# wen-yuan-zhang/Fast-Learning-NeRF

Measured on AMD Instinct MI355X. Metric: training rays/sec (Lego-like 800x800, 64+128 samples) + PSNR@N-iters, higher is better.
Workload: dtype f32; 1 GPU; nerf-ours Lego full 800x800 (BASELINE configs[1]), SURVEY 8(d) throughput protocol: 4096 uniformly drawn rays per GPU per step, 64+128 samples, use_viewdirs, white_bkgd, perturb=1, U[0,1) targets, random-init nets, leaf-error table on, fp32-width bf16x6 kernels, plain backward (FASTNERF_COMPACT=0); parallelism=dp1, math_mode=bf16x6, backward=plain (every sample)

## Files before the change

fast-learning-nerf_amd/csrc/mlp_bwd_dw.hip:

```cpp
#include "mlp_common.h"
#include "dw_pair.h"
#include <atomic>

int fn_launch_dx(int mm, int grid, hipStream_t st, int64_t P, const float* draw, const float* act, const float* params, const float* packed_bwd,
                 float* dact, const NetLayout& L, const int* live_idx, const int* live_cnt, float* headws, int flags);

#define DW_MT 32

template <int WO, int WI, int TO, int TI, bool BIAS, bool RANK1>
__global__ void __launch_bounds__(WO * WI * 64, WO * WI / 4)
mlp_bwd_dw_kernel(int64_t P, const float* __restrict__ dY, int ldy, const float* __restrict__ X, int ldx,
                  const float* __restrict__ draw , float* __restrict__ partial_w,
                  float* __restrict__ partial_b, float* __restrict__ partial_r, const int* __restrict__ live_idx,
                  const int* __restrict__ live_cnt) {
  if (live_idx) P = (int64_t)__builtin_amdgcn_readfirstlane(*live_cnt);
  constexpr int NO = WO * TO * 32, KI = WI * TI * 32;
  constexpr int NTD = WO * WI * 64;
  constexpr int STAGE = DW_MT * (NO + KI) + DW_MT;
  extern __shared__ __attribute__((aligned(16))) float smem[];
  const int tid = threadIdx.x;
  const int lane = tid & 63;
  const int wave = __builtin_amdgcn_readfirstlane(tid >> 6);
  const int wo = wave / WI, wi = wave % WI;
  const int64_t ntile_all = (P + DW_MT - 1) / DW_MT;
  const int64_t per = (ntile_all + gridDim.x - 1) / gridDim.x;
  const int64_t t0 = blockIdx.x * per;
  int64_t t1 = t0 + per;
  if (t1 > ntile_all) t1 = ntile_all;

  f32x16 acc[TO][TI];
#pragma unroll
  for (int a = 0; a < TO; ++a)
#pragma unroll
    for (int b = 0; b < TI; ++b)
#pragma unroll
      for (int r = 0; r < 16; ++r) acc[a][b][r] = 0.f;
  float bsum = 0.f, rsum = 0.f;

  constexpr int YV = (DW_MT * NO / 4 + NTD - 1) / NTD;
  constexpr int XV = (DW_MT * KI / 4 + NTD - 1) / NTD;
  static_assert(DW_MT * NO % 4 == 0 && DW_MT * KI % 4 == 0 && NO <= NTD && KI <= NTD, "stage split");
  float4 ry[YV], rx[XV];
  float rda = 0.f;

  auto load_stage = [&](int64_t t) {
    const int64_t pbase = t * DW_MT;
#pragma unroll
    for (int i = 0; i < YV; ++i) {
      const int e = (i * NTD + tid) * 4;
      const int m = e / NO, c = e % NO;
      const int64_t p = pbase + m;
      ry[i] = (e < DW_MT * NO && p < P) ? *reinterpret_cast<const float4*>(dY + p * ldy + c)
                                        : make_float4(0.f, 0.f, 0.f, 0.f);
    }
#pragma unroll
    for (int i = 0; i < XV; ++i) {
      const int e = (i * NTD + tid) * 4;
      const int m = e / KI, c = e % KI;
      const int64_t p = pbase + m;
      rx[i] = (e < DW_MT * KI && p < P) ? *reinterpret_cast<const float4*>(X + p * ldx + c)
                                        : make_float4(0.f, 0.f, 0.f, 0.f);
    }
    if (RANK1 && tid < DW_MT) {
      const int64_t p = pbase + tid;
      rda = (p < P) ? draw[(live_idx ? (int64_t)live_idx[p] : p) * 4 + 3] : 0.f;
    }
  };
  auto store_stage = [&](float* st) {
#pragma unroll
    for (int i = 0; i < YV; ++i)
      if ((i * NTD + tid) * 4 < DW_MT * NO) *reinterpret_cast<float4*>(st + (i * NTD + tid) * 4) = ry[i];
#pragma unroll
    for (int i = 0; i < XV; ++i)
      if ((i * NTD + tid) * 4 < DW_MT * KI) *reinterpret_cast<float4*>(st + DW_MT * NO + (i * NTD + tid) * 4) = rx[i];
    if (RANK1 && tid < DW_MT) st[DW_MT * (NO + KI) + tid] = rda;
  };

  if (t0 < t1) {
    load_stage(t0);
    store_stage(smem);
  }
  __syncthreads();
  for (int64_t t = t0; t < t1; ++t) {
    float* cur = smem + ((t - t0) & 1) * STAGE;
    float* nxt = smem + (((t - t0) & 1) ^ 1) * STAGE;
    if (t + 1 < t1) load_stage(t + 1);
    const float* Ys = cur;
    const float* Xs = cur + DW_MT * NO;
    {
      float fa0[TO], fb0[TI], fa1[TO], fb1[TI];
      auto ldf = [&](float (&a)[TO], float (&b)[TI], int k2) {
        const int m = k2 * 2 + (lane >> 5);
#pragma unroll
        for (int i = 0; i < TO; ++i) a[i] = Ys[m * NO + (wo * TO + i) * 32 + (lane & 31)];
#pragma unroll
        for (int j = 0; j < TI; ++j) b[j] = Xs[m * KI + (wi * TI + j) * 32 + (lane & 31)];
      };
      auto mm = [&](const float (&a)[TO], const float (&b)[TI]) {
#pragma unroll
        for (int i = 0; i < TO; ++i)
#pragma unroll
          for (int j = 0; j < TI; ++j) acc[i][j] = mfma(a[i], b[j], acc[i][j]);
      };
      ldf(fa0, fb0, 0);
#pragma unroll
      for (int k2 = 0; k2 < DW_MT / 2; k2 += 2) {
        ldf(fa1, fb1, k2 + 1);
        __builtin_amdgcn_sched_barrier(0);
        mm(fa0, fb0);
        __builtin_amdgcn_sched_barrier(0);
        if (k2 + 2 < DW_MT / 2) ldf(fa0, fb0, k2 + 2);
        __builtin_amdgcn_sched_barrier(0);
        mm(fa1, fb1);
        __builtin_amdgcn_sched_barrier(0);
      }
    }
    if (BIAS) {
      if (tid < NO) {
#pragma unroll 8
        for (int m = 0; m < DW_MT; ++m) bsum += Ys[m * NO + tid];
      }
    }
    if (RANK1) {
      if (tid < KI) {
        const float* da = cur + DW_MT * (NO + KI);
#pragma unroll 8
        for (int m = 0; m < DW_MT; ++m) rsum = fmaf(da[m], Xs[m * KI + tid], rsum);
      }
    }
    if (t + 1 < t1) store_stage(nxt);
    __syncthreads();
  }
  float* pw = partial_w + (int64_t)blockIdx.x * NO * KI;
#pragma unroll
  for (int i = 0; i < TO; ++i)
#pragma unroll
    for (int j = 0; j < TI; ++j)
#pragma unroll
      for (int r = 0; r < 16; ++r) {
        const int o = (wo * TO + i) * 32 + crow(r, lane);
        const int c = (wi * TI + j) * 32 + (lane & 31);
        pw[(int64_t)o * KI + c] = acc[i][j][r];
      }
  if (BIAS && tid < NO) partial_b[(int64_t)blockIdx.x * NO + tid] = bsum;
  if (RANK1 && tid < KI) partial_r[(int64_t)blockIdx.x * KI + tid] = rsum;
}

template <int WO, int WI, int TO, int TI, bool BIAS, bool RANK1, int CTI2 = 0, int CTO2 = 0, bool RBV = false>
__device__ __forceinline__ void dw6_body(const int64_t P, const float* __restrict__ dY, const float* __restrict__ X,
                                         const float* __restrict__ draw, float* __restrict__ partial_w, float* __restrict__ partial_b,
                                         float* __restrict__ partial_r, const int* __restrict__ live_idx,
                                         const float* __restrict__ X2, const float* __restrict__ dY2, const int wg, const int nwg,
                                         const float* __restrict__ rb_wr = nullptr) {
  constexpr int NO = WO * TO * 32, KI = WI * TI * 32;
  constexpr int CTO = WO * TO, CTI = WI * TI, NTILE = CTO + CTI;
  constexpr int NW = WO * WI;
  constexpr int TPW = (NTILE + NW - 1) / NW;
  extern __shared__ __attribute__((aligned(16))) uint4 S6[];
  float* const DA = reinterpret_cast<float*>(S6 + 2 * NTILE * 192);
  float4* const DR = reinterpret_cast<float4*>(DA + 32);
  static_assert(!RBV || (RANK1 && CTO2 == 0), "the view job: draw is staged, one gradient tensor");
  const int tid = threadIdx.x;
  const int lane = tid & 63;
  const int wave = __builtin_amdgcn_readfirstlane(tid >> 6);
  const int wo = wave / WI, wi = wave % WI;
  const int64_t nq_all = (P + 15) / 16;
  const int64_t per = (nq_all + nwg - 1) / nwg;
  const int64_t q0 = wg * per;
  int64_t q1 = q0 + per;
  if (q1 > nq_all) q1 = nq_all;
  const int nq = (int)(q1 - q0);
  int64_t Pend = q1 * 16;
  if (Pend > P) Pend = P;

  f32x16 acc[TO][TI];
#pragma unroll
  for (int a = 0; a < TO; ++a)
#pragma unroll
    for (int b = 0; b < TI; ++b)
#pragma unroll
      for (int r = 0; r < 16; ++r) acc[a][b][r] = 0.f;
  float ssum[TPW];
#pragma unroll
  for (int k = 0; k < TPW; ++k) ssum[k] = 0.f;

  constexpr int CTI1 = CTI - CTI2, KI1 = CTI1 * 32, KI2 = CTI2 * 32;
  constexpr int CTO1 = CTO - CTO2, NO1 = CTO1 * 32, NO2 = CTO2 * 32;
  static_assert(!(RANK1 && CTO2) && !(CTI2 && CTO2), "one second tensor per job");
  const float* tsrc[TPW];
  bool tisy[TPW], tis2[TPW];
  constexpr bool KNOWN = (CTO % NW == 0) && (NTILE % NW == 0) && CTO2 == 0 && CTI2 == 0;
#pragma unroll
  for (int k = 0; k < TPW; ++k) {
    const int t = k * NW + wave;
    tisy[k] = KNOWN ? (k * NW < CTO) : (t < CTO);
    tis2[k] = (CTI2 > 0 && t >= CTO + CTI1) || (CTO2 > 0 && t >= CTO1 && t < CTO);
    tsrc[k] = tisy[k] ? (tis2[k] ? dY2 + q0 * (16 * NO2) + (t - CTO1) * 32 : dY + q0 * (16 * NO1) + t * 32)
                      : (tis2[k] ? X2 + q0 * (16 * KI2) + (t - CTO - CTI1) * 32 : X + q0 * (16 * KI1) + (t - CTO) * 32);
  }
  const int relmax = (int)(Pend - q0 * 16) - 1;
  const int col = lane & 31, half8 = (lane >> 5) * 8;
  const unsigned boffy = (unsigned)(half8 * NO1 + col) * 4u, boffy2 = (unsigned)(half8 * NO2 + col) * 4u,
                 boffx = (unsigned)(half8 * KI1 + col) * 4u, boffx2 = (unsigned)(half8 * KI2 + col) * 4u;
  struct Raw { float v[TPW][8]; };
  float wr0[TPW], wr1[TPW], wr2[TPW];
  if constexpr (RBV) {
#pragma unroll
    for (int k = 0; k < TPW; ++k) {
      const int t = k * NW + wave;
      if (tisy[k] && (NTILE % NW == 0 || t < NTILE)) {
        wr0[k] = rb_wr[t * 32 + col]; wr1[k] = rb_wr[128 + t * 32 + col]; wr2[k] = rb_wr[256 + t * 32 + col];
      } else {
        wr0[k] = wr1[k] = wr2[k] = 0.f;
      }
    }
  }
  auto ldb = [](const float* base, unsigned byte_off) __attribute__((always_inline)) -> float {
    return *reinterpret_cast<const float*>(reinterpret_cast<const char*>(base) + byte_off);
  };
  auto load_raw = [&](Raw& r, int st, auto whole) __attribute__((always_inline)) {
    if constexpr (decltype(whole)::value) {
#pragma unroll
      for (int k = 0; k < TPW; ++k) {
        const int t = k * NW + wave;
        if (NTILE % NW == 0 || t < NTILE) {
          if (tisy[k] && CTO2 > 0 && tis2[k]) {
            const float* b = tsrc[k] + (int64_t)st * (16 * NO2);
#pragma unroll
            for (int e = 0; e < 8; ++e) r.v[k][e] = ldb(b, boffy2 + (unsigned)(e * NO2 * 4));
          } else if (tisy[k]) {
            const float* b = tsrc[k] + (int64_t)st * (16 * NO1);
#pragma unroll
            for (int e = 0; e < 8; ++e) r.v[k][e] = ldb(b, boffy + (unsigned)(e * NO1 * 4));
          } else if (CTI2 > 0 && tis2[k]) {
            const float* b = tsrc[k] + (int64_t)st * (16 * KI2);
#pragma unroll
            for (int e = 0; e < 8; ++e) r.v[k][e] = ldb(b, boffx2 + (unsigned)(e * KI2 * 4));
          } else {
            const float* b = tsrc[k] + (int64_t)st * (16 * KI1);
#pragma unroll
            for (int e = 0; e < 8; ++e) r.v[k][e] = ldb(b, boffx + (unsigned)(e * KI1 * 4));
          }
        }
      }
    } else {
      unsigned row[8];
#pragma unroll
      for (int e = 0; e < 8; ++e) { const int rr = st * 16 + half8 + e; row[e] = (unsigned)(rr < relmax ? rr : relmax); }
#pragma unroll
      for (int k = 0; k < TPW; ++k) {
        const int t = k * NW + wave;
        if (NTILE % NW == 0 || t < NTILE) {
#pragma unroll
          for (int e = 0; e < 8; ++e)
            r.v[k][e] = ldb(tsrc[k], (row[e] * (unsigned)(tisy[k] ? (tis2[k] ? NO2 : NO1) : (tis2[k] ? KI2 : KI1)) + (unsigned)col) * 4u);
        }
      }
    }
  };
  const int* const li = live_idx ? live_idx : reinterpret_cast<const int*>(draw);
  auto load_ix = [&](int st) __attribute__((always_inline)) -> int64_t {
    const int rr = st * 16 + (lane & 15);
    const int64_t p = q0 * 16 + (rr < relmax ? rr : relmax);
    const int64_t lv = li[p];
    return live_idx ? lv : p;
  };
  auto split_store = [&](const Raw& r, int buf, int st, auto whole) __attribute__((always_inline)) {
    const int nv = relmax + 1 - (st * 16 + half8);
#pragma unroll
    for (int k = 0; k < TPW; ++k) {
      const int t = k * NW + wave;
      if (NTILE % NW == 0 || t < NTILE) {
        float v[8];
#pragma unroll
        for (int e = 0; e < 8; ++e) v[e] = r.v[k][e];
        if constexpr (RBV) {
          if (tisy[k]) {
#pragma unroll
            for (int e = 0; e < 8; ++e) {
              const float4 d = DR[(st & 1) * 16 + half8 + e];
              v[e] = dyv_value(v[e], d.x, d.y, d.z, wr0[k], wr1[k], wr2[k]);
            }
          }
        }
        if constexpr (!decltype(whole)::value) {
#pragma unroll
          for (int e = 0; e < 8; ++e) v[e] = e < nv ? v[e] : 0.f;
        }
        uint4 h, m, l;
        uint4* d = S6 + ((buf * NTILE + t) * 3) * 64 + lane;
        split3_frag(make_float4(v[0], v[1], v[2], v[3]), make_float4(v[4], v[5], v[6], v[7]), h, m, l);
        d[0] = h; d[64] = m; d[128] = l;
        if (BIAS && (KNOWN ? (k * NW < CTO) : (t < CTO1))) ssum[k] += ((v[0] + v[1]) + (v[2] + v[3])) + ((v[4] + v[5]) + (v[6] + v[7]));
        if (RANK1 && (KNOWN ? (k * NW >= CTO) : (t >= CTO && t < CTO + CTI1))) {
          const float4 d0 = *reinterpret_cast<const float4*>(DA + (st & 1) * 16 + half8);
          const float4 d1 = *reinterpret_cast<const float4*>(DA + (st & 1) * 16 + half8 + 4);
          const float da[8] = {d0.x, d0.y, d0.z, d0.w, d1.x, d1.y, d1.z, d1.w};
#pragma unroll
          for (int e = 0; e < 8; ++e) ssum[k] = fmaf(da[e], v[e], ssum[k]);
        }
      }
    }
  };
  auto multiply = [&](int buf) __attribute__((always_inline)) {
    const uint4* Sb = S6 + buf * NTILE * 192 + lane;
    uint4 a[TO][3];
#pragma unroll
    for (int i = 0; i < TO; ++i)
#pragma unroll
      for (int pl = 0; pl < 3; ++pl) a[i][pl] = Sb[((wo * TO + i) * 3 + pl) * 64];
    constexpr int PA[6] = {2, 0, 1, 1, 0, 0}, PB[6] = {0, 2, 1, 0, 1, 0};
    constexpr int JP = TI >= 2 ? 2 : 1;
#pragma unroll
    for (int j0 = 0; j0 < TI; j0 += JP) {
      uint4 b[JP][3];
#pragma unroll
      for (int jj = 0; jj < JP; ++jj)
#pragma unroll
        for (int pl = 0; pl < 3; ++pl)
          if (j0 + jj < TI) b[jj][pl] = Sb[((CTO + wi * TI + j0 + jj) * 3 + pl) * 64];
#pragma unroll
      for (int t = 0; t < 6; ++t)
#pragma unroll
        for (int jj = 0; jj < JP; ++jj)
#pragma unroll
          for (int i = 0; i < TO; ++i)
            if (j0 + jj < TI) acc[i][j0 + jj] = mfma_bf16(a[i][PA[t]], b[jj][PB[t]], acc[i][j0 + jj]);
    }
  };
  auto publish = [&]() __attribute__((always_inline)) {
    asm volatile("s_waitcnt lgkmcnt(0)\n\ts_barrier" ::: "memory");
  };

  if (nq > 0) {
    constexpr std::true_type WHOLE{};
    constexpr std::false_type ANY{};
    Raw r0, r1;
    load_raw(r0, 0, ANY);
    load_raw(r1, 1, ANY);
    typedef typename std::conditional<RBV, float4, float>::type DrawT;
    auto ld_draw = [&](int64_t ix) __attribute__((always_inline)) -> DrawT {
      if constexpr (RBV) return *reinterpret_cast<const float4*>(draw + ix * 4);
      else return draw[ix * 4 + 3];
    };
    auto st_draw = [&](int slot, const DrawT& d) __attribute__((always_inline)) {
      if constexpr (RBV) { DA[slot] = d.w; DR[slot] = d; }
      else DA[slot] = d;
    };
    DrawT dr0 = DrawT(), dr1 = DrawT();
    int64_t ix0 = 0, ix1 = 0;
    const bool da_lane = RANK1 && wave == 0 && lane < 16;
    if (da_lane) {
      st_draw(lane, ld_draw(load_ix(0)));
      st_draw(16 + lane, ld_draw(load_ix(1)));
      dr0 = ld_draw(load_ix(2));
      dr1 = ld_draw(load_ix(3));
      ix0 = load_ix(4);
      ix1 = load_ix(5);
    }
    if (RANK1) publish();
    split_store(r0, 0, 0, ANY);
    load_raw(r0, 2, ANY);
    publish();
    auto mix = [&](auto sync) __attribute__((always_inline)) {
      if constexpr (KNOWN && !RANK1) interleave6<0, TO * TI * 6, TPW * 4 * 11 + (BIAS ? 8 : 0), decltype(sync)::value>();
    };
    auto pair = [&](int d, auto whole) __attribute__((always_inline)) {
      const int st = 2 * d;
      if (da_lane) { st_draw(lane, dr0); dr0 = ld_draw(ix0); ix0 = load_ix(st + 6); }
      multiply(0);
      split_store(r1, 1, st + 1, whole);
      mix(std::integral_constant<int, 1>{});
      load_raw(r1, st + 3, whole);
      publish();
      if (da_lane) { st_draw(16 + lane, dr1); dr1 = ld_draw(ix1); ix1 = load_ix(st + 7); }
      multiply(1);
      split_store(r0, 0, st + 2, whole);
      mix(std::integral_constant<int, 2>{});
      load_raw(r0, st + 4, whole);
      publish();
    };
    const int n2 = (nq + 1) / 2;
    const int nwhole = (relmax + 1) / 16;
    int dmain = nwhole >= 5 ? (nwhole - 3) / 2 : 0;
    if (dmain > n2) dmain = n2;
#pragma unroll 1
    for (int d = 0; d < dmain; ++d) pair(d, WHOLE);
#pragma unroll 1
    for (int d = dmain; d < n2; ++d) pair(d, ANY);
  }
  float* pw = partial_w + (int64_t)wg * NO * KI;
#pragma unroll
  for (int i = 0; i < TO; ++i)
#pragma unroll
    for (int j = 0; j < TI; ++j)
#pragma unroll
      for (int r = 0; r < 16; ++r) {
        const int o = (wo * TO + i) * 32 + crow(r, lane);
        const int c = (wi * TI + j) * 32 + (lane & 31);
        pw[(int64_t)o * KI + c] = acc[i][j][r];
      }
  if (BIAS || RANK1) {
#pragma unroll
    for (int k = 0; k < TPW; ++k) {
      const int t = k * NW + wave;
      if (NTILE % NW == 0 || t < NTILE) {
        const float sv = ssum[k] + __shfl_xor(ssum[k], 32, 64);
        if (lane < 32) {
          if (BIAS && t < CTO1) partial_b[(int64_t)wg * NO1 + t * 32 + lane] = sv;
          if (RANK1 && t >= CTO && t < CTO + CTI1) partial_r[(int64_t)wg * KI1 + (t - CTO) * 32 + lane] = sv;
        }
      }
    }
  }
}

template <int WO, int WI, int TO, int TI, bool BIAS, bool RANK1, int CTI2 = 0, int CTO2 = 0>
__global__ void __launch_bounds__(WO * WI * 64, WO * WI / 4)
mlp_bwd_dw6_kernel(int64_t P, const float* __restrict__ dY, const float* __restrict__ X,
                   const float* __restrict__ draw, float* __restrict__ partial_w, float* __restrict__ partial_b,
                   float* __restrict__ partial_r, const int* __restrict__ live_idx, const int* __restrict__ live_cnt,
                   const float* __restrict__ X2 = nullptr, const float* __restrict__ dY2 = nullptr) {
  if (live_idx) P = (int64_t)__builtin_amdgcn_readfirstlane(*live_cnt);
  dw6_body<WO, WI, TO, TI, BIAS, RANK1, CTI2, CTO2>(P, dY, X, draw, partial_w, partial_b, partial_r, live_idx, X2, dY2, (int)blockIdx.x,
                                                    (int)gridDim.x);
}

template <int WO, int WI, int TO, int TI, bool BIAS, bool RANK1, int CTI2>
__global__ void __launch_bounds__(WO * WI * 64, WO * WI / 4)
mlp_bwd_dw6_rbv_kernel(int64_t P, const float* __restrict__ hv, const float* __restrict__ X, const float* __restrict__ draw,
                       float* __restrict__ partial_w, float* __restrict__ partial_b, float* __restrict__ partial_r,
                       const float* __restrict__ X2, const float* __restrict__ wr) {
  dw6_body<WO, WI, TO, TI, BIAS, RANK1, CTI2, 0, true>(P, hv, X, draw, partial_w, partial_b, partial_r, nullptr, X2, nullptr, (int)blockIdx.x,
                                                       (int)gridDim.x, wr);
}

#define DW_QMAX 256
__host__ __device__ static inline int dw_trunk_chunks(int64_t P, int ncu) {
  const int unit = ncu >= 8 ? ncu / 8 : 1;
  const int64_t nq = (P + 15) / 16;
  int64_t k = (nq + (int64_t)unit * DW_QMAX - 1) / ((int64_t)unit * DW_QMAX);
  k = k < 1 ? 1 : (k > 8 ? 8 : k);
  return unit * (int)k;
}
__global__ void __launch_bounds__(512, 2)
mlp_bwd_dw6_trunk_kernel(int64_t P, DwTrunk J, const int* __restrict__ live_idx, const int* __restrict__ live_cnt, int ncu) {
  if (live_idx) P = (int64_t)__builtin_amdgcn_readfirstlane(*live_cnt);
  const int nact = dw_trunk_chunks(P, ncu);
  if ((int)blockIdx.x >= nact) return;
  const int job = (int)blockIdx.y;
  dw6_body<4, 2, 2, 4, true, false>(P, J.dY[job], J.X[job], nullptr, J.pw[job], J.pb[job], nullptr, live_idx, nullptr, nullptr,
                                    (int)blockIdx.x, nact);
}

struct DwTrunkPair {
  DwTrunk J[2];
  int64_t P[2];
};
__global__ void __launch_bounds__(512, 2)
mlp_bwd_dw6_trunk_pair_kernel(DwTrunkPair A, int ncu) {
  const int c0 = dw_trunk_chunks(A.P[0], ncu);
  int b = (int)blockIdx.x;
  const int pass = b >= DW_TRUNK_JOBS * c0 ? 1 : 0;
  if (pass) b -= DW_TRUNK_JOBS * c0;
  const int64_t P = A.P[pass];
  const int nact = pass ? dw_trunk_chunks(P, ncu) : c0;
  const int job = b / nact;
  if (job >= DW_TRUNK_JOBS) return;
  const DwTrunk& J = A.J[pass];
  dw6_body<4, 2, 2, 4, true, false>(P, J.dY[job], J.X[job], nullptr, J.pw[job], J.pb[job], nullptr, nullptr, nullptr, nullptr, b - job * nact,
                                    nact);
}

__global__ void __launch_bounds__(128) head_grads_kernel(int64_t P, const float* __restrict__ draw,
                                                          const float* __restrict__ hv,
                                                          float* __restrict__ partial, const int* __restrict__ live_idx,
                                                          const int* __restrict__ live_cnt) {
  const int k = threadIdx.x;
  if (live_idx) P = *live_cnt;
  auto dptr = [&](int64_t q) { return draw + (live_idx ? (int64_t)live_idx[q] : q) * 4; };
  const int64_t per = (P + gridDim.x - 1) / gridDim.x;
  const int64_t pa = blockIdx.x * per;
  int64_t pb = pa + per;
  if (pb > P) pb = P;
  float s0 = 0.f, s1 = 0.f, s2 = 0.f, sb = 0.f;
  int64_t p = pa;
  constexpr int NF = 16;
  for (; p + NF <= pb; p += NF) {
    float4 d[NF];
    float h[NF];
#pragma unroll
    for (int i = 0; i < NF; ++i) {
      d[i] = *reinterpret_cast<const float4*>(dptr(p + i));
      h[i] = hv[(p + i) * 128 + k];
    }
#pragma unroll
    for (int i = 0; i < NF; ++i) {
      s0 = fmaf(d[i].x, h[i], s0); s1 = fmaf(d[i].y, h[i], s1); s2 = fmaf(d[i].z, h[i], s2);
      if (k < 4) sb += (k == 0) ? d[i].x : (k == 1) ? d[i].y : (k == 2) ? d[i].z : d[i].w;
    }
  }
  for (; p < pb; ++p) {
    const float4 d = *reinterpret_cast<const float4*>(dptr(p));
    const float h = hv[p * 128 + k];
    s0 = fmaf(d.x, h, s0); s1 = fmaf(d.y, h, s1); s2 = fmaf(d.z, h, s2);
    if (k < 4) sb += (k == 0) ? d.x : (k == 1) ? d.y : (k == 2) ? d.z : d.w;
  }
  float* o = partial + (int64_t)blockIdx.x * 388;
  o[k] = s0; o[128 + k] = s1; o[256 + k] = s2;
  if (k < 4) o[384 + k] = sb;
}

#define HEAD_ROWS 256
__host__ __device__ static inline int head_group(int64_t ntiles) {
  const int64_t g = (ntiles + HEAD_ROWS - 1) / HEAD_ROWS;
  return g < 1 ? 1 : (int)g;
}
__host__ __device__ static inline int head_rows(int64_t P) {
  const int64_t ntiles = (P + TM - 1) / TM;
  const int g = head_group(ntiles);
  return (int)((ntiles + g - 1) / g);
}
__global__ void __launch_bounds__(128) head_group_kernel(int64_t P, const float* __restrict__ ws, float* __restrict__ out,
                                                          const int* __restrict__ live_cnt) {
  if (live_cnt) P = (int64_t)*live_cnt;
  const int64_t ntiles = (P + TM - 1) / TM;
  const int g = head_group(ntiles);
  const int col = (int)blockIdx.y * 128 + (int)threadIdx.x;
  const int64_t t0 = (int64_t)blockIdx.x * g;
  if (t0 >= ntiles || col >= 388) return;
  const int n = (int)(ntiles - t0 < g ? ntiles - t0 : g);
  const float* src = ws + t0 * 388 + col;
  constexpr int NF = 16;
  float s = 0.f;
  int i = 0;
  for (; i + NF <= n; i += NF) {
    float v[NF];
#pragma unroll
    for (int j = 0; j < NF; ++j) v[j] = src[(int64_t)(i + j) * 388];
#pragma unroll
    for (int j = 0; j < NF; ++j) s += v[j];
  }
  for (; i < n; ++i) s += src[(int64_t)i * 388];
  out[(int64_t)blockIdx.x * 388 + col] = s;
}


__global__ void __launch_bounds__(256) reduce_all_kernel(RedTable tab, const float* __restrict__ partial, float* __restrict__ grads,
                                                          float* __restrict__ scratch, int64_t P, const int* __restrict__ live_cnt, int ncu) {
  RedSeg sg = tab.s[blockIdx.y];
  if (sg.dyn) {
    if (live_cnt) P = (int64_t)*live_cnt;
    const int n = sg.dyn == 2 ? head_rows(P) : dw_trunk_chunks(P, ncu);
    sg.nwg = n < sg.nwg ? n : sg.nwg;
  }
  const int64_t total = (int64_t)sg.rows * sg.cols;
  const float* src = partial + sg.src;
  for (int64_t e = blockIdx.x * (int64_t)blockDim.x + threadIdx.x; e < total; e += (int64_t)gridDim.x * blockDim.x) {
    const int r = (int)(e / sg.cols), c = (int)(e % sg.cols);
    if (c >= sg.valid_cols) continue;
    constexpr int RS = 16;
    float a[RS];
#pragma unroll
    for (int i = 0; i < RS; ++i) a[i] = 0.f;
    int w = 0;
    for (; w + RS <= sg.nwg; w += RS) {
#pragma unroll
      for (int i = 0; i < RS; ++i) a[i] += src[(int64_t)(w + i) * sg.wg_stride + e];
    }
#pragma unroll
    for (int i = 0; i < RS - 1; ++i)
      if (w + i < sg.nwg) a[i] += src[(int64_t)(w + i) * sg.wg_stride + e];
#pragma unroll
    for (int h = RS / 2; h >= 1; h >>= 1)
#pragma unroll
      for (int i = 0; i < h; ++i) a[i] += a[i + h];
    if (c < sg.sc_cols) scratch[sg.sc_dst + (int64_t)r * sg.sc_cols + c] = a[0];
    else grads[sg.dst + (int64_t)r * sg.ld + c] = a[0];
  }
}

__global__ void __launch_bounds__(256) unfold_kernel(const float* __restrict__ G, const float* __restrict__ params, float* __restrict__ grads,
                                                      int64_t VW, int64_t VB, int64_t FW, int64_t FB) {
  __shared__ double As[16][17], Bs[16][17];
  const int tx = threadIdx.x & 15, ty = threadIdx.x >> 4;
  const int b = blockIdx.x;
  if (b == 384) {
    const int i = threadIdx.x;
    double s = 0.0;
    for (int o = 0; o < 128; ++o) s = fma((double)params[VW + (int64_t)o * 283 + i], (double)grads[VB + o], s);
    grads[FB + i] = (float)s;
    return;
  }
  const bool wf = b < 256;
  const int r0 = wf ? (b >> 4) * 16 : ((b - 256) >> 4) * 16, c0 = (b & 15) * 16;
  const int K = wf ? 128 : 256;
  double s = 0.0;
  for (int k0 = 0; k0 < K; k0 += 16) {
    if (wf) {
      As[ty][tx] = (double)params[VW + (int64_t)(k0 + ty) * 283 + r0 + tx];
      Bs[ty][tx] = (double)G[(k0 + ty) * 256 + c0 + tx];
    } else {
      As[tx][ty] = (double)G[(r0 + ty) * 256 + k0 + tx];
      Bs[tx][ty] = (double)params[FW + (int64_t)(c0 + ty) * 256 + k0 + tx];
    }
    __syncthreads();
#pragma unroll
    for (int k = 0; k < 16; ++k) s = fma(As[k][ty], Bs[k][tx], s);
    __syncthreads();
  }
  if (wf) grads[FW + (int64_t)(r0 + ty) * 256 + c0 + tx] = (float)s;
  else grads[VW + (int64_t)(r0 + ty) * 283 + c0 + tx] = (float)fma((double)grads[VB + r0 + ty], (double)params[FB + c0 + tx], s);
}

extern "C" int64_t fastnerf_mlp_bwd_partial_floats(void) {
  return dw_partial_floats(fn::device_cus());
}

template <int WO, int WI, int TO, int TI, bool BIAS, bool RANK1, int MM = MM_F32, int CTI2 = 0, int CTO2 = 0>
static int launch_dw(int64_t P, const float* dY, int ldy, const float* X, int ldx, const float* draw, float* base,
                     int nwg, hipStream_t st, const int* live_idx = nullptr, const int* live_cnt = nullptr,
                     const float* X2 = nullptr, const float* dY2 = nullptr, float* pr_at = nullptr) {
  constexpr int NO = WO * TO * 32, KI = WI * TI * 32;
  float* pw = base;
  float* pb = base + (int64_t)nwg * NO * KI;
  float* pr = pr_at ? pr_at : pb + (BIAS ? (int64_t)nwg * (NO - CTO2 * 32) : 0);
  if constexpr (MM == MM_X6) {
    if (ldy != NO - CTO2 * 32 || ldx != KI - CTI2 * 32 || (CTI2 > 0) != (X2 != nullptr) || (CTO2 > 0) != (dY2 != nullptr)) {
      fn::set_error("launch_dw: the bf16x6 dW kernel needs ld == width (and X2 / dY2 exactly when CTI2 / CTO2 > 0)");
      return -1;
    }
    constexpr int lds6 = 2 * (WO * TO + WI * TI) * 3 * 1024 + 128;
    auto kern6 = mlp_bwd_dw6_kernel<WO, WI, TO, TI, BIAS, RANK1, CTI2, CTO2>;
    static fn::DevOnce once6;
    if (int rc = fn::set_dyn_lds(reinterpret_cast<const void*>(kern6), once6, lds6)) return rc;
    hipLaunchKernelGGL(kern6, dim3(nwg), dim3(WO * WI * 64), lds6, st, P, dY, X, draw, pw, pb, pr, live_idx, live_cnt, X2, dY2);
    FN_LAUNCH_CHECK();
    return 0;
  } else {
    static_assert(MM == MM_F32 && CTI2 == 0 && CTO2 == 0, "two-tensor jobs exist for the bf16x6 dW kernel only");
    constexpr int STAGE = DW_MT * (NO + KI) + DW_MT;
    const size_t lds = 2 * STAGE * sizeof(float);
    auto kern = mlp_bwd_dw_kernel<WO, WI, TO, TI, BIAS, RANK1>;
    static fn::DevOnce once;
    if (int rc = fn::set_dyn_lds(reinterpret_cast<const void*>(kern), once, (int)lds)) return rc;
    hipLaunchKernelGGL(kern, dim3(nwg), dim3(WO * WI * 64), lds, st, P, dY, ldy, X, ldx, draw, pw, pb, pr, live_idx, live_cnt);
    FN_LAUNCH_CHECK();
    return 0;
  }
}

template <int WO, int WI, int TO, int TI, bool BIAS, bool RANK1, int CTI2>
static int launch_dw_rbv(int64_t P, const float* hv, const float* X, const float* draw, float* base, int nwg, hipStream_t st, const float* X2,
                         float* pr_at, const float* wr) {
  constexpr int NO = WO * TO * 32, KI = WI * TI * 32;
  float* pw = base;
  float* pb = base + (int64_t)nwg * NO * KI;
  float* pr = pr_at ? pr_at : pb + (BIAS ? (int64_t)nwg * NO : 0);
  constexpr int lds6 = 2 * (WO * TO + WI * TI) * 3 * 1024 + 128 + 512;
  auto kern = mlp_bwd_dw6_rbv_kernel<WO, WI, TO, TI, BIAS, RANK1, CTI2>;
  static fn::DevOnce once;
  if (int rc = fn::set_dyn_lds(reinterpret_cast<const void*>(kern), once, lds6)) return rc;
  hipLaunchKernelGGL(kern, dim3(nwg), dim3(WO * WI * 64), lds6, st, P, hv, X, draw, pw, pb, pr, X2, wr);
  FN_LAUNCH_CHECK();
  return 0;
}

static void add_seg(RedTable& T, int64_t src, int64_t wg_stride, int nwg, int rows, int cols, int64_t dst, int ld,
                    int valid_cols, int dyn = 0, int sc_cols = 0, int64_t sc_dst = 0) {
  RedSeg& s = T.s[T.n++];
  s.src = src; s.wg_stride = wg_stride; s.nwg = nwg; s.rows = rows; s.cols = cols; s.dst = dst; s.ld = ld;
  s.valid_cols = valid_cols; s.dyn = dyn; s.sc_cols = sc_cols; s.sc_dst = sc_dst;
}

constexpr int DW_TRUNK_LDS = 2 * 16 * 3 * 1024 + 128;
static int trunk_chunks_fit(int64_t P, int ncu, int nwg) {
  if (dw_trunk_chunks(P, ncu) > nwg) {
    fn::set_error("mlp_bwd: the trunk launch needs %d chunks per job, the partial regions hold %d (a device with fewer than 8 CUs?)",
                  dw_trunk_chunks(P, ncu), nwg);
    return -1;
  }
  return 0;
}

static int bwd_reduce(const RedTable& T, const NetLayout& L, int64_t P, const float* params, float* partial, float* grads, int64_t g_off,
                      const int* live_cnt, int ncu, hipStream_t st) {
  hipLaunchKernelGGL(reduce_all_kernel, dim3(256, T.n), dim3(256), 0, st, T, partial, grads, partial, P, live_cnt, ncu);
  FN_LAUNCH_CHECK();
  hipLaunchKernelGGL(unfold_kernel, dim3(385), dim3(256), 0, st, partial + g_off, params, grads, L.VW, L.VB, L.FW, L.FB);
  FN_LAUNCH_CHECK();
  return 0;
}

namespace fn {
static float* head_workspace(int64_t ntiles, hipStream_t st) {
  const char* e = getenv("FASTNERF_HEAD_FROM_DX");
  if (e && e[0] == '0') return nullptr;
  static const WsName what = {
      "fastnerf: no memory for the per-tile head partials of the backward (%.1f MB): this stream keeps the head_grads launch\n", 1e-6};
  const StreamWs w = stream_ws(WS_HEAD_TILES, st, (ntiles > 0 ? ntiles : 1) * 388, what);
  if (w.p && e && e[0] == 'n') (void)hipMemsetAsync(w.p, 0xFF, sizeof(float) * (size_t)w.cap, st);
  return w.p;
}
}

static std::atomic<int64_t> g_rebuild_passes{0};
namespace fn {
int side_rebuild_mode(void) {
  const char* e = getenv("FASTNERF_SIDE_REBUILD");
  if (e && e[0] == '0') return 0;
  return (e && e[0] == 'n') ? 2 : 1;
}
}

template <int MM>
static int bwd_launch_t(int kind, int64_t n, int S, const float* draw, const float* act, const float* params,
                      const float* packed_bwd, float* dact, float* partial, float* grads, const int* live_idx,
                      const int* live_cnt, fn_stream_t stream, DwDeferred* defer = nullptr, const SideRb* rb = nullptr) {
  constexpr int MW = MM;
  const NetLayout& L = layout_of(kind);
  const int PEP = L.pe_pad;
  hipStream_t st = fn::S(stream);
  const int64_t P = n * S;
  const int64_t ntiles = (P + TM - 1) / TM;
  const int ncu = fn::device_cus();
  int grid = ncu * WG_PER_CU;
  if (ntiles < grid) grid = (int)ntiles;
  float* const headws = fn::head_workspace(ntiles, st);
  if (rb && (MM != MM_X6 || PEP != 64 || live_idx)) {
    fn::set_error("mlp_bwd: the rebuilding view job needs bf16x6, the 64-channel encoding and no live list");
    return -1;
  }
  if (rb) g_rebuild_passes.fetch_add(1, std::memory_order_relaxed);
  if (rb && rb->poison) (void)hipMemsetAsync(dact + dact_yv(P), 0xFF, sizeof(float) * (size_t)P * 128, st);
  if (int rc_dx = fn_launch_dx(MM, grid, st, P, draw, act, params, packed_bwd, dact, L, live_idx, live_cnt, headws,
                               (rb && rb->no_store) ? FN_DX_NO_DYV_STORE : 0))
    return rc_dx;

  const int nwg = ncu;
  RedTable T;
  T.n = 0;
  int rc;
  const float* a_pe = act + act_pe(P, PEP);
  auto region = [&](int j) { return partial + dw_job_base(j, ncu, PEP); };
  auto segs = [&](int j, int64_t dstW, int ld, int validc, int64_t dstB, int64_t dstR, int dyn = 0) {
    const DwJobDesc d = dw_job(j, PEP);
    const int64_t b = dw_job_base(j, ncu, PEP);
    add_seg(T, b, (int64_t)d.NO * d.KI, nwg, d.NO, d.KI, dstW, ld, validc, dyn);
    int64_t o = b + (int64_t)nwg * d.NO * d.KI;
    if (d.bias) { add_seg(T, o, d.NO, nwg, 1, d.NO, dstB, d.NO, d.NO, dyn); o += (int64_t)nwg * d.NO; }
    if (d.rank1) add_seg(T, o, d.KI, nwg, 1, d.KI, dstR, d.KI, d.KI, dyn);
  };
  if constexpr (MW == MM_X6) {
    if (PEP == 64) rc = launch_dw<8, 2, 2, 1, true, false, MW, 0, 8>(P, dact + dact_y(P, 0), 256, a_pe, 64, nullptr, region(0), nwg, st, live_idx, live_cnt, nullptr, dact + dact_y(P, 5));
    else rc = launch_dw<8, 1, 2, 3, true, false, MW, 0, 8>(P, dact + dact_y(P, 0), 256, a_pe, 96, nullptr, region(0), nwg, st, live_idx, live_cnt, nullptr, dact + dact_y(P, 5));
    if (rc) return rc;
    const int64_t b0 = dw_job_base(0, ncu, PEP);
    add_seg(T, b0, (int64_t)512 * PEP, nwg, 256, PEP, L.LW[0], L.in_pe, L.in_pe);
    add_seg(T, b0 + (int64_t)256 * PEP, (int64_t)512 * PEP, nwg, 256, PEP, L.LW[5], 256 + L.in_pe, L.in_pe);
    add_seg(T, b0 + (int64_t)nwg * 512 * PEP, 256, nwg, 1, 256, L.LB[0], 256, 256);
  } else {
    if (PEP == 64) rc = launch_dw<4, 1, 2, 2, true, false, MW>(P, dact + dact_y(P, 0), 256, a_pe, 64, nullptr, region(0), nwg, st, live_idx, live_cnt);
    else rc = launch_dw<4, 1, 2, 3, true, false, MW>(P, dact + dact_y(P, 0), 256, a_pe, 96, nullptr, region(0), nwg, st, live_idx, live_cnt);
    if (rc) return rc;
    segs(0, L.LW[0], L.in_pe, L.in_pe, L.LB[0], 0);
  }
  if constexpr (MW != MM_X6) {
    for (int l = 1; l < 8; ++l) {
      if ((rc = launch_dw<4, 2, 2, 4, true, false, MW>(P, dact + dact_y(P, l), 256, act + act_h(P, PEP, l - 1), 256, nullptr, region(l), nwg, st, live_idx, live_cnt))) return rc;
      segs(l, L.LW[l] + (l == 5 ? L.in_pe : 0), l == 5 ? 256 + L.in_pe : 256, 256, L.LB[l], 0);
    }
  }
  if constexpr (MW != MM_X6) {
    if (PEP == 64) rc = launch_dw<4, 1, 2, 2, false, false, MW>(P, dact + dact_y(P, 5), 256, a_pe, 64, nullptr, region(8), nwg, st, live_idx, live_cnt);
    else rc = launch_dw<4, 1, 2, 3, false, false, MW>(P, dact + dact_y(P, 5), 256, a_pe, 96, nullptr, region(8), nwg, st, live_idx, live_cnt);
    if (rc) return rc;
    segs(8, L.LW[5], 256 + L.in_pe, L.in_pe, 0, 0);
  }
  if constexpr (MW == MM_X6) {
    DwTrunk J;
    for (int l = 1; l < 8; ++l) {
      J.dY[l - 1] = dact + dact_y(P, l);
      J.X[l - 1] = act + act_h(P, PEP, l - 1);
      J.pw[l - 1] = region(l);
      J.pb[l - 1] = region(l) + (int64_t)nwg * 256 * 256;
    }
    if ((rc = trunk_chunks_fit(P, ncu, nwg))) return rc;
    if (defer) {
      defer->J = J;
    } else {
      static fn::DevOnce once_t;
      if ((rc = fn::set_dyn_lds(reinterpret_cast<const void*>(mlp_bwd_dw6_trunk_kernel), once_t, DW_TRUNK_LDS))) return rc;
      hipLaunchKernelGGL(mlp_bwd_dw6_trunk_kernel, dim3(dw_trunk_chunks(P, ncu), DW_TRUNK_JOBS), dim3(512), DW_TRUNK_LDS, st, P, J, live_idx, live_cnt, ncu);
      FN_LAUNCH_CHECK();
    }
    for (int l = 1; l < 8; ++l) segs(l, L.LW[l] + (l == 5 ? L.in_pe : 0), l == 5 ? 256 + L.in_pe : 256, 256, L.LB[l], 0, 1);
  }
  float* const pr_view = region(9);
  const int64_t g_off = dw_job_base(9, ncu, PEP) + (int64_t)nwg * 256;
  if constexpr (MW == MM_X6) {
    if (rb) rc = launch_dw_rbv<4, 3, 1, 3, true, true, 1>(P, act + act_hv(P, PEP), act + act_h(P, PEP, 7), draw, region(10), nwg, st, act + act_vpe(P, PEP),
                                                          pr_view, params + L.RW);
    else rc = launch_dw<4, 3, 1, 3, true, true, MW, 1, 0>(P, dact + dact_yv(P), 128, act + act_h(P, PEP, 7), 256, draw, region(10), nwg, st,
                                                    live_idx, live_cnt, act + act_vpe(P, PEP), nullptr, pr_view);
    if (rc) return rc;
    const int64_t b10 = dw_job_base(10, ncu, PEP);
    add_seg(T, b10, 128 * 288, nwg, 128, 288, L.VW, 283, 283, 0, 256, g_off);
    add_seg(T, b10 + (int64_t)nwg * 128 * 288, 128, nwg, 1, 128, L.VB, 128, 128);
  } else {
    if ((rc = launch_dw<2, 4, 2, 2, true, true, MW>(P, dact + dact_yv(P), 128, act + act_h(P, PEP, 7), 256, draw, region(10), nwg, st, live_idx, live_cnt,
                                              nullptr, nullptr, pr_view))) return rc;
    const int64_t b10 = dw_job_base(10, ncu, PEP);
    add_seg(T, b10, 128 * 256, nwg, 128, 256, L.VW, 283, 256, 0, 256, g_off);
    add_seg(T, b10 + (int64_t)nwg * 128 * 256, 128, nwg, 1, 128, L.VB, 128, 128);
    if ((rc = launch_dw<4, 1, 1, 1, false, false, MW>(P, dact + dact_yv(P), 128, act + act_vpe(P, PEP), 32, nullptr, region(11), nwg, st, live_idx, live_cnt))) return rc;
    segs(11, L.VW + 256, 283, 27, 0, 0);
  }
  add_seg(T, dw_job_base(9, ncu, PEP), 256, nwg, 1, 256, L.AW, 256, 256);
  if (headws != nullptr) {
    const int64_t hb = dw_job_base(12, ncu, PEP);
    const int rows = ntiles < HEAD_ROWS ? (int)ntiles : HEAD_ROWS;
    hipLaunchKernelGGL(head_group_kernel, dim3(rows, 4), dim3(128), 0, st, P, headws, partial + hb, live_cnt);
    FN_LAUNCH_CHECK();
    add_seg(T, hb, 388, rows, 1, 388, L.RW, 388, 387, 2);
    add_seg(T, hb + 387, 388, rows, 1, 1, L.AB, 1, 1, 2);
  } else {
    const int hg = HEAD_MAX_WG;
    const int64_t hb = dw_job_base(12, ncu, PEP);
    hipLaunchKernelGGL(head_grads_kernel, dim3(hg), dim3(128), 0, st, P, draw, act + act_hv(P, PEP), partial + hb, live_idx, live_cnt);
    FN_LAUNCH_CHECK();
    add_seg(T, hb, 388, hg, 1, 388, L.RW, 388, 387);
    add_seg(T, hb + 387, 388, hg, 1, 1, L.AB, 1, 1);
  }
  if (defer) {
    defer->T = T; defer->P = P; defer->g_off = g_off; defer->params = params; defer->partial = partial; defer->grads = grads; defer->kind = kind;
    return 0;
  }
  return bwd_reduce(T, L, P, params, partial, grads, g_off, live_cnt, ncu, st);
}

namespace fn {
static std::atomic<int64_t> g_pair_launches{0};

bool x6_pair_workspace(int64_t P_coarse, fn_stream_t stream, float** dact2, float** partial2) {
  static const WsName what = {
      "fastnerf: no memory for the side workspace of the paired bf16x6 backward (%.2f GB): this stream keeps the per-pass trunk launches\n", 1e-9};
  const StreamWs d = stream_ws(WS_PAIR_DACT, S(stream), P_coarse * (int64_t)DACT_FLOATS, what);
  if (!d.p) return false;
  const StreamWs p = stream_ws(WS_PAIR_PARTIAL, S(stream), fastnerf_mlp_bwd_partial_floats(), what);
  if (!p.p) return false;
  *dact2 = d.p;
  *partial2 = p.p;
  return true;
}

int x6_pair_pass(DwDeferred* d, int64_t n, int S, const float* draw, const float* act, const float* params, const float* packed_bwd,
                 float* dact, float* partial, float* grads, fn_stream_t stream, const SideRb* rb) {
  FN_CHECK_ARG(d && n > 0 && S >= 1, "d != NULL, n>0, S>=1");
  FN_CHECK_ARG(draw && act && params && packed_bwd && dact && partial && grads, "null pointer");
  return bwd_launch_t<MM_X6>(0, n, S, draw, act, params, packed_bwd, dact, partial, grads, nullptr, nullptr, stream, d, rb);
}
int x6_bwd_rebuild(int64_t n, int S, const float* draw, const float* act, const float* params, const float* packed_bwd, float* dact,
                   float* partial, float* grads, fn_stream_t stream, const SideRb* rb) {
  FN_CHECK_ARG(n > 0 && S >= 1 && rb, "n>0, S>=1, rb != NULL");
  FN_CHECK_ARG(draw && act && params && packed_bwd && dact && partial && grads, "null pointer");
  return bwd_launch_t<MM_X6>(0, n, S, draw, act, params, packed_bwd, dact, partial, grads, nullptr, nullptr, stream, nullptr, rb);
}

int x6_pair_finish(const DwDeferred* fine, const DwDeferred* coarse, fn_stream_t stream) {
  hipStream_t st = S(stream);
  const int ncu = fn::device_cus();
  const DwDeferred* d[2] = {fine, coarse};
  DwTrunkPair A;
  int nwg = 0;
  for (int k = 0; k < 2; ++k) {
    A.J[k] = d[k]->J;
    A.P[k] = d[k]->P;
    nwg += DW_TRUNK_JOBS * dw_trunk_chunks(A.P[k], ncu);
  }
  static DevOnce once_p;
  if (int rc = set_dyn_lds(reinterpret_cast<const void*>(mlp_bwd_dw6_trunk_pair_kernel), once_p, DW_TRUNK_LDS)) return rc;
  hipLaunchKernelGGL(mlp_bwd_dw6_trunk_pair_kernel, dim3(nwg), dim3(512), DW_TRUNK_LDS, st, A, ncu);
  FN_LAUNCH_CHECK();
  g_pair_launches.fetch_add(1, std::memory_order_relaxed);
  for (int k = 0; k < 2; ++k)
    if (int rc = bwd_reduce(d[k]->T, layout_of(d[k]->kind), d[k]->P, d[k]->params, d[k]->partial, d[k]->grads, d[k]->g_off, nullptr, ncu, st)) return rc;
  return 0;
}
}
extern "C" int64_t fastnerf_x6_pair_launches(void) { return fn::g_pair_launches.load(std::memory_order_relaxed); }
extern "C" int64_t fastnerf_side_rebuild_passes(void) { return g_rebuild_passes.load(std::memory_order_relaxed); }

static int bwd_launch(int kind, int64_t n, int S, const float* draw, const float* act, const float* params,
                      const float* packed_bwd, float* dact, float* partial, float* grads, const int* live_idx,
                      const int* live_cnt, fn_stream_t stream, int mm = MM_F32) {
  return mm == MM_X6 ? bwd_launch_t<MM_X6>(kind, n, S, draw, act, params, packed_bwd, dact, partial, grads, live_idx, live_cnt, stream)
                     : bwd_launch_t<MM_F32>(kind, n, S, draw, act, params, packed_bwd, dact, partial, grads, live_idx, live_cnt, stream);
}
extern "C" int fastnerf_mlp_bwd_ex(int kind, int64_t n, int S, const float* draw, const float* act,
                                   const float* params, const float* packed_bwd, float* dact, float* partial,
                                   float* grads, fn_stream_t stream) {
  FN_CHECK_ARG(kind >= 0 && kind <= 2 && n > 0 && S >= 1, "kind in 0..2, n>0, S>=1");
  FN_CHECK_ARG(draw && act && params && packed_bwd && dact && partial && grads, "null pointer");
  return bwd_launch(kind, n, S, draw, act, params, packed_bwd, dact, partial, grads, nullptr, nullptr, stream);
}
extern "C" int fastnerf_mlp_bwd_live_ex(int kind, int64_t n, int S, const float* draw, const float* act,
                                        const float* params, const float* packed_bwd, float* dact, float* partial,
                                        float* grads, const int32_t* live_idx, const int32_t* live_cnt,
                                        fn_stream_t stream) {
  FN_CHECK_ARG(kind >= 0 && kind <= 2 && n > 0 && S >= 1, "kind in 0..2, n>0, S>=1");
  FN_CHECK_ARG(draw && act && params && packed_bwd && dact && partial && grads && live_idx && live_cnt, "null pointer");
  return bwd_launch(kind, n, S, draw, act, params, packed_bwd, dact, partial, grads, live_idx, live_cnt, stream);
}
extern "C" int fastnerf_mlp_bwd(int64_t n, int S, const float* draw, const float* act, const float* params,
                                const float* packed_bwd, float* dact, float* partial, float* grads,
                                fn_stream_t stream) {
  return fastnerf_mlp_bwd_ex(0, n, S, draw, act, params, packed_bwd, dact, partial, grads, stream);
}

extern "C" int fastnerf_mlp_x6_bwd(int kind, int64_t n, int S, const float* draw, const float* act, const float* params,
                                   const float* packed_bwd, float* dact, float* partial, float* grads, fn_stream_t stream) {
  FN_CHECK_ARG(kind >= 0 && kind <= 2 && n > 0 && S >= 1, "kind in 0..2, n>0, S>=1");
  FN_CHECK_ARG(draw && act && params && packed_bwd && dact && partial && grads, "null pointer");
  return bwd_launch(kind, n, S, draw, act, params, packed_bwd, dact, partial, grads, nullptr, nullptr, stream, MM_X6);
}
extern "C" int fastnerf_mlp_x6_bwd_live(int kind, int64_t n, int S, const float* draw, const float* act, const float* params,
                                        const float* packed_bwd, float* dact, float* partial, float* grads,
                                        const int32_t* live_idx, const int32_t* live_cnt, fn_stream_t stream) {
  FN_CHECK_ARG(kind >= 0 && kind <= 2 && n > 0 && S >= 1, "kind in 0..2, n>0, S>=1");
  FN_CHECK_ARG(draw && act && params && packed_bwd && dact && partial && grads && live_idx && live_cnt, "null pointer");
  return bwd_launch(kind, n, S, draw, act, params, packed_bwd, dact, partial, grads, live_idx, live_cnt, stream, MM_X6);
}
```

Before: 251,500 rays/s.

## Specialize view-layer dW kernel waves by role to drop per-wave tile branching

For the view-direction weight-gradient jobs, where the tile count is one more than the wave count, each wave is now compiled as one of four role-specialized bodies. Each role carries only one or two tiles, so most waves stop allocating registers for a second, mostly idle tile slot, and the draw-staging lane becomes a dedicated role. Scheduling barriers and role-tuned interleave counts are added around loads and split stores on the tail path and in the main loop. This adds code size through four instantiations and risks register or schedule imbalance across waves.

```diff
diff --git a/fast-learning-nerf_amd/csrc/mlp_bwd_dw.hip b/fast-learning-nerf_amd/csrc/mlp_bwd_dw.hip
--- a/fast-learning-nerf_amd/csrc/mlp_bwd_dw.hip
+++ b/fast-learning-nerf_amd/csrc/mlp_bwd_dw.hip
@@ -146,7 +146,10 @@
   if (RANK1 && tid < KI) partial_r[(int64_t)blockIdx.x * KI + tid] = rsum;
 }
 
-template <int WO, int WI, int TO, int TI, bool BIAS, bool RANK1, int CTI2 = 0, int CTO2 = 0, bool RBV = false>
+constexpr int dw6_role_valu(int role, bool rbv) {
+  return 18 * (role == 0 ? (rbv ? 6 : 4) : role == 1 ? (rbv ? 6 : 3) : role == 2 ? 8 : 4);
+}
+template <int WO, int WI, int TO, int TI, bool BIAS, bool RANK1, int CTI2 = 0, int CTO2 = 0, bool RBV = false, int ROLE = -1>
 __device__ __forceinline__ void dw6_body(const int64_t P, const float* __restrict__ dY, const float* __restrict__ X,
                                          const float* __restrict__ draw, float* __restrict__ partial_w, float* __restrict__ partial_b,
                                          float* __restrict__ partial_r, const int* __restrict__ live_idx,
@@ -155,7 +158,9 @@
   constexpr int NO = WO * TO * 32, KI = WI * TI * 32;
   constexpr int CTO = WO * TO, CTI = WI * TI, NTILE = CTO + CTI;
   constexpr int NW = WO * WI;
-  constexpr int TPW = (NTILE + NW - 1) / NW;
+  constexpr bool ROLED = ROLE >= 0;
+  static_assert(!ROLED || (ROLE < 4 && NTILE == NW + 1 && CTO < NW && CTI2 == 1 && CTO2 == 0 && BIAS && RANK1), "roles: the view jobs");
+  constexpr int TPW = ROLED ? (ROLE == 2 ? 2 : 1) : (NTILE + NW - 1) / NW;
   extern __shared__ __attribute__((aligned(16))) uint4 S6[];
   float* const DA = reinterpret_cast<float*>(S6 + 2 * NTILE * 192);
   float4* const DR = reinterpret_cast<float4*>(DA + 32);
@@ -190,11 +195,13 @@
   const float* tsrc[TPW];
   bool tisy[TPW], tis2[TPW];
   constexpr bool KNOWN = (CTO % NW == 0) && (NTILE % NW == 0) && CTO2 == 0 && CTI2 == 0;
+#define DW6_TILE(k) (ROLED ? ((k) == 0 ? wave : NTILE - 1) : (k) * NW + wave)
+  constexpr bool ALLT = ROLED || NTILE % NW == 0;
 #pragma unroll
   for (int k = 0; k < TPW; ++k) {
-    const int t = k * NW + wave;
-    tisy[k] = KNOWN ? (k * NW < CTO) : (t < CTO);
-    tis2[k] = (CTI2 > 0 && t >= CTO + CTI1) || (CTO2 > 0 && t >= CTO1 && t < CTO);
+    const int t = DW6_TILE(k);
+    tisy[k] = ROLED ? (ROLE < 2) : KNOWN ? (k * NW < CTO) : (t < CTO);
+    tis2[k] = ROLED ? (k == 1) : ((CTI2 > 0 && t >= CTO + CTI1) || (CTO2 > 0 && t >= CTO1 && t < CTO));
     tsrc[k] = tisy[k] ? (tis2[k] ? dY2 + q0 * (16 * NO2) + (t - CTO1) * 32 : dY + q0 * (16 * NO1) + t * 32)
                       : (tis2[k] ? X2 + q0 * (16 * KI2) + (t - CTO - CTI1) * 32 : X + q0 * (16 * KI1) + (t - CTO) * 32);
   }
@@ -207,8 +214,8 @@
   if constexpr (RBV) {
 #pragma unroll
     for (int k = 0; k < TPW; ++k) {
-      const int t = k * NW + wave;
-      if (tisy[k] && (NTILE % NW == 0 || t < NTILE)) {
+      const int t = DW6_TILE(k);
+      if (tisy[k] && (ALLT || t < NTILE)) {
         wr0[k] = rb_wr[t * 32 + col]; wr1[k] = rb_wr[128 + t * 32 + col]; wr2[k] = rb_wr[256 + t * 32 + col];
       } else {
         wr0[k] = wr1[k] = wr2[k] = 0.f;
@@ -222,8 +229,8 @@
     if constexpr (decltype(whole)::value) {
 #pragma unroll
       for (int k = 0; k < TPW; ++k) {
-        const int t = k * NW + wave;
-        if (NTILE % NW == 0 || t < NTILE) {
+        const int t = DW6_TILE(k);
+        if (ALLT || t < NTILE) {
           if (tisy[k] && CTO2 > 0 && tis2[k]) {
             const float* b = tsrc[k] + (int64_t)st * (16 * NO2);
 #pragma unroll
@@ -249,8 +256,8 @@
       for (int e = 0; e < 8; ++e) { const int rr = st * 16 + half8 + e; row[e] = (unsigned)(rr < relmax ? rr : relmax); }
 #pragma unroll
       for (int k = 0; k < TPW; ++k) {
-        const int t = k * NW + wave;
-        if (NTILE % NW == 0 || t < NTILE) {
+        const int t = DW6_TILE(k);
+        if (ALLT || t < NTILE) {
 #pragma unroll
           for (int e = 0; e < 8; ++e)
             r.v[k][e] = ldb(tsrc[k], (row[e] * (unsigned)(tisy[k] ? (tis2[k] ? NO2 : NO1) : (tis2[k] ? KI2 : KI1)) + (unsigned)col) * 4u);
@@ -259,8 +266,9 @@
     }
   };
   const int* const li = live_idx ? live_idx : reinterpret_cast<const int*>(draw);
+  const int dl = lane & 15;
   auto load_ix = [&](int st) __attribute__((always_inline)) -> int64_t {
-    const int rr = st * 16 + (lane & 15);
+    const int rr = st * 16 + dl;
     const int64_t p = q0 * 16 + (rr < relmax ? rr : relmax);
     const int64_t lv = li[p];
     return live_idx ? lv : p;
@@ -269,8 +277,8 @@
     const int nv = relmax + 1 - (st * 16 + half8);
 #pragma unroll
     for (int k = 0; k < TPW; ++k) {
-      const int t = k * NW + wave;
-      if (NTILE % NW == 0 || t < NTILE) {
+      const int t = DW6_TILE(k);
+      if (ALLT || t < NTILE) {
         float v[8];
 #pragma unroll
         for (int e = 0; e < 8; ++e) v[e] = r.v[k][e];
@@ -291,8 +299,8 @@
         uint4* d = S6 + ((buf * NTILE + t) * 3) * 64 + lane;
         split3_frag(make_float4(v[0], v[1], v[2], v[3]), make_float4(v[4], v[5], v[6], v[7]), h, m, l);
         d[0] = h; d[64] = m; d[128] = l;
-        if (BIAS && (KNOWN ? (k * NW < CTO) : (t < CTO1))) ssum[k] += ((v[0] + v[1]) + (v[2] + v[3])) + ((v[4] + v[5]) + (v[6] + v[7]));
-        if (RANK1 && (KNOWN ? (k * NW >= CTO) : (t >= CTO && t < CTO + CTI1))) {
+        if (BIAS && (ROLED ? tisy[k] : KNOWN ? (k * NW < CTO) : (t < CTO1))) ssum[k] += ((v[0] + v[1]) + (v[2] + v[3])) + ((v[4] + v[5]) + (v[6] + v[7]));
+        if (RANK1 && (ROLED ? (!tisy[k] && !tis2[k]) : KNOWN ? (k * NW >= CTO) : (t >= CTO && t < CTO + CTI1))) {
           const float4 d0 = *reinterpret_cast<const float4*>(DA + (st & 1) * 16 + half8);
           const float4 d1 = *reinterpret_cast<const float4*>(DA + (st & 1) * 16 + half8 + 4);
           const float da[8] = {d0.x, d0.y, d0.z, d0.w, d1.x, d1.y, d1.z, d1.w};
@@ -336,8 +344,11 @@
     constexpr std::true_type WHOLE{};
     constexpr std::false_type ANY{};
     Raw r0, r1;
+    auto fence = [&]() __attribute__((always_inline)) { if constexpr (ROLED) __builtin_amdgcn_sched_barrier(0); };
     load_raw(r0, 0, ANY);
+    fence();
     load_raw(r1, 1, ANY);
+    fence();
     typedef typename std::conditional<RBV, float4, float>::type DrawT;
     auto ld_draw = [&](int64_t ix) __attribute__((always_inline)) -> DrawT {
       if constexpr (RBV) return *reinterpret_cast<const float4*>(draw + ix * 4);
@@ -349,10 +360,10 @@
     };
     DrawT dr0 = DrawT(), dr1 = DrawT();
     int64_t ix0 = 0, ix1 = 0;
-    const bool da_lane = RANK1 && wave == 0 && lane < 16;
+    const bool da_lane = ROLED ? (ROLE == 0) : (RANK1 && wave == 0 && lane < 16);
     if (da_lane) {
-      st_draw(lane, ld_draw(load_ix(0)));
-      st_draw(16 + lane, ld_draw(load_ix(1)));
+      st_draw(dl, ld_draw(load_ix(0)));
+      st_draw(16 + dl, ld_draw(load_ix(1)));
       dr0 = ld_draw(load_ix(2));
       dr1 = ld_draw(load_ix(3));
       ix0 = load_ix(4);
@@ -360,23 +371,29 @@
     }
     if (RANK1) publish();
     split_store(r0, 0, 0, ANY);
+    fence();
     load_raw(r0, 2, ANY);
     publish();
-    auto mix = [&](auto sync) __attribute__((always_inline)) {
+    auto mix = [&](auto sync, auto whole) __attribute__((always_inline)) {
       if constexpr (KNOWN && !RANK1) interleave6<0, TO * TI * 6, TPW * 4 * 11 + (BIAS ? 8 : 0), decltype(sync)::value>();
+      if constexpr (ROLED && decltype(whole)::value) interleave6<0, TO * TI * 6, dw6_role_valu(ROLE, RBV), decltype(sync)::value>();
     };
     auto pair = [&](int d, auto whole) __attribute__((always_inline)) {
       const int st = 2 * d;
-      if (da_lane) { st_draw(lane, dr0); dr0 = ld_draw(ix0); ix0 = load_ix(st + 6); }
+      if (da_lane) { st_draw(dl, dr0); dr0 = ld_draw(ix0); ix0 = load_ix(st + 6); }
       multiply(0);
+      if constexpr (!decltype(whole)::value) fence();
       split_store(r1, 1, st + 1, whole);
-      mix(std::integral_constant<int, 1>{});
+      mix(std::integral_constant<int, 1>{}, whole);
+      if constexpr (!decltype(whole)::value) fence();
       load_raw(r1, st + 3, whole);
       publish();
-      if (da_lane) { st_draw(16 + lane, dr1); dr1 = ld_draw(ix1); ix1 = load_ix(st + 7); }
+      if (da_lane) { st_draw(16 + dl, dr1); dr1 = ld_draw(ix1); ix1 = load_ix(st + 7); }
       multiply(1);
+      if constexpr (!decltype(whole)::value) fence();
       split_store(r0, 0, st + 2, whole);
-      mix(std::integral_constant<int, 2>{});
+      mix(std::integral_constant<int, 2>{}, whole);
+      if constexpr (!decltype(whole)::value) fence();
       load_raw(r0, st + 4, whole);
       publish();
     };
@@ -403,8 +420,8 @@
   if (BIAS || RANK1) {
 #pragma unroll
     for (int k = 0; k < TPW; ++k) {
-      const int t = k * NW + wave;
-      if (NTILE % NW == 0 || t < NTILE) {
+      const int t = DW6_TILE(k);
+      if (ALLT || t < NTILE) {
         const float sv = ssum[k] + __shfl_xor(ssum[k], 32, 64);
         if (lane < 32) {
           if (BIAS && t < CTO1) partial_b[(int64_t)wg * NO1 + t * 32 + lane] = sv;
@@ -413,6 +430,24 @@
       }
     }
   }
+}
+
+#undef DW6_TILE
+
+constexpr bool dw6_has_roles(int WO, int WI, int TO, int TI, bool BIAS, bool RANK1, int CTI2, int CTO2) {
+  return BIAS && RANK1 && CTI2 == 1 && CTO2 == 0 && WO * TO + WI * TI == WO * WI + 1 && WO * TO < WO * WI;
+}
+template <int WO, int WI, int TO, int TI, bool RBV>
+__device__ __forceinline__ void dw6_view_roles(const int64_t P, const float* __restrict__ dY, const float* __restrict__ X,
+                                               const float* __restrict__ draw, float* __restrict__ partial_w, float* __restrict__ partial_b,
+                                               float* __restrict__ partial_r, const int* __restrict__ live_idx,
+                                               const float* __restrict__ X2, const float* __restrict__ wr) {
+  const int wave = __builtin_amdgcn_readfirstlane(threadIdx.x >> 6);
+  const int wg = (int)blockIdx.x, nwg = (int)gridDim.x;
+  if (wave == 0) dw6_body<WO, WI, TO, TI, true, true, 1, 0, RBV, 0>(P, dY, X, draw, partial_w, partial_b, partial_r, live_idx, X2, nullptr, wg, nwg, wr);
+  else if (wave < WO * TO) dw6_body<WO, WI, TO, TI, true, true, 1, 0, RBV, 1>(P, dY, X, draw, partial_w, partial_b, partial_r, live_idx, X2, nullptr, wg, nwg, wr);
+  else if (wave == WO * TO) dw6_body<WO, WI, TO, TI, true, true, 1, 0, RBV, 2>(P, dY, X, draw, partial_w, partial_b, partial_r, live_idx, X2, nullptr, wg, nwg, wr);
+  else dw6_body<WO, WI, TO, TI, true, true, 1, 0, RBV, 3>(P, dY, X, draw, partial_w, partial_b, partial_r, live_idx, X2, nullptr, wg, nwg, wr);
 }
 
 template <int WO, int WI, int TO, int TI, bool BIAS, bool RANK1, int CTI2 = 0, int CTO2 = 0>
@@ -422,8 +457,11 @@
                    float* __restrict__ partial_r, const int* __restrict__ live_idx, const int* __restrict__ live_cnt,
                    const float* __restrict__ X2 = nullptr, const float* __restrict__ dY2 = nullptr) {
   if (live_idx) P = (int64_t)__builtin_amdgcn_readfirstlane(*live_cnt);
-  dw6_body<WO, WI, TO, TI, BIAS, RANK1, CTI2, CTO2>(P, dY, X, draw, partial_w, partial_b, partial_r, live_idx, X2, dY2, (int)blockIdx.x,
-                                                    (int)gridDim.x);
+  if constexpr (dw6_has_roles(WO, WI, TO, TI, BIAS, RANK1, CTI2, CTO2))
+    dw6_view_roles<WO, WI, TO, TI, false>(P, dY, X, draw, partial_w, partial_b, partial_r, live_idx, X2, nullptr);
+  else
+    dw6_body<WO, WI, TO, TI, BIAS, RANK1, CTI2, CTO2>(P, dY, X, draw, partial_w, partial_b, partial_r, live_idx, X2, dY2, (int)blockIdx.x,
+                                                      (int)gridDim.x);
 }
 
 template <int WO, int WI, int TO, int TI, bool BIAS, bool RANK1, int CTI2>
@@ -431,8 +469,8 @@
 mlp_bwd_dw6_rbv_kernel(int64_t P, const float* __restrict__ hv, const float* __restrict__ X, const float* __restrict__ draw,
                        float* __restrict__ partial_w, float* __restrict__ partial_b, float* __restrict__ partial_r,
                        const float* __restrict__ X2, const float* __restrict__ wr) {
-  dw6_body<WO, WI, TO, TI, BIAS, RANK1, CTI2, 0, true>(P, hv, X, draw, partial_w, partial_b, partial_r, nullptr, X2, nullptr, (int)blockIdx.x,
-                                                       (int)gridDim.x, wr);
+  static_assert(dw6_has_roles(WO, WI, TO, TI, BIAS, RANK1, CTI2, 0), "the rebuilding job is a view job");
+  dw6_view_roles<WO, WI, TO, TI, true>(P, hv, X, draw, partial_w, partial_b, partial_r, nullptr, X2, wr);
 }
 
 #define DW_QMAX 256
```

Result: no change. 252,200 rays/s, median of 6 (+0.3%).
